# XuyangBai/PointDSC

Measured on NVIDIA H100. Metric: correspondence-sets/sec (PointDSC.forward, N=1000, B=256), higher is better.
Workload: dtype fp16 hi/lo split (3 products) with f32 accumulate

## Files before the change

pointdsc_b200/csrc/tc_attention.cuh:

```cuda
#pragma once
#include "tc_common.cuh"

namespace pdsc {

struct AttnArgs {
  int split;
  const uint8_t* qimg;
  const uint8_t* kvimg;
  const float* sc;
  float* msg;
  int items;
  float* part_o;
  float* part_ml;
  const SetDesc* sets;
  int nsets;
};

struct AttnItem {
  int N, QT, KT;
  int qt, t0, T;
  int sp;
  int qtile, kt0;
  int row0;
  long long sc0;
};

__device__ __forceinline__ AttnItem attn_item(const AttnArgs& a, int witem) {
  const SetDesc d = a.sets[find_set(a.nsets, witem, [&](int i) { return a.sets[i].item0; })];
  const int local = witem - d.item0;
  AttnItem w;
  w.N = d.N; w.QT = (d.N + 127) / 128; w.KT = (d.N + 63) / 64;
  w.qt = local / d.sp; w.t0 = (local % d.sp) * d.TS; w.T = d.TS; w.sp = d.sp;
  w.qtile = d.qt0 + w.qt; w.kt0 = d.kt0; w.row0 = d.row0; w.sc0 = d.sc0;
  return w;
}

constexpr int kAttnThreads = 384;
constexpr uint32_t kAttnConsumerRegs = 232, kAttnProducerRegs = 40;

__device__ __forceinline__ float ex2_approx(float x) {
  float y;
  asm("ex2.approx.ftz.f32 %0, %1;" : "=f"(y) : "f"(x));
  return y;
}
__device__ __forceinline__ float2 ldg_stream2(const float* p) {
  float2 v;
  asm volatile("ld.global.nc.L1::no_allocate.v2.f32 {%0, %1}, [%2];" : "=f"(v.x), "=f"(v.y) : "l"(p));
  return v;
}
__device__ __forceinline__ void attn_load_sc(float (&sc)[32], const float* tile, int r0, int fc) {
#pragma unroll
  for (int jj = 0; jj < 8; ++jj)
#pragma unroll
    for (int h = 0; h < 2; ++h) {
      const int key = 8 * jj + fc;
      const float2 v = ldg_stream2(tile + ((key >> 2) * 128 + r0 + 8 * h) * 4 + (key & 3));
      sc[4 * jj + 2 * h] = v.x;
      sc[4 * jj + 2 * h + 1] = v.y;
    }
}

}
```

pointdsc_b200/csrc/tc_attention_p.cuh:

```cuda
#pragma once
#include "tc_attention.cuh"

namespace pdsc {

constexpr int kAttnPQ = 0;
constexpr int kAttnPKV = 65536;
constexpr int kAttnStages = 2;
constexpr int kAttnPBars = kAttnPKV + kAttnStages * 65536;
constexpr int kAttnPSmem = kAttnPBars + 128;

template <int FMT>
__global__ void __launch_bounds__(kAttnThreads, 1) tc_attention_persistent_kernel(AttnArgs a) {
  extern __shared__ __align__(1024) uint8_t smem[];
  uint64_t* bars = reinterpret_cast<uint64_t*>(smem + kAttnPBars);
  const uint32_t s0 = smem_u32(smem);
  const uint32_t q_full = smem_u32(bars + 0), q_empty = smem_u32(bars + 1);
  const uint32_t kv_full = smem_u32(bars + 2), kv_empty = smem_u32(bars + 4);
  const int tid = threadIdx.x, warp = tid >> 5, lane = tid & 31;
  const int my_items = (a.items > (int)blockIdx.x) ? (a.items - (int)blockIdx.x + (int)gridDim.x - 1) / (int)gridDim.x : 0;

  if (tid == 0) {
    if (s0 & 1023u) __trap();
    mbar_init(q_full, 1);
    mbar_init(q_empty, 256);
    for (int i = 0; i < kAttnStages; ++i) {
      mbar_init(kv_full + 8 * i, 1);
      mbar_init(kv_empty + 8 * i, 256);
    }
    fence_barrier_init();
  }
  __syncthreads();

  if (warp >= 8) {
    setmaxnreg_dec<kAttnProducerRegs>();
    if (warp == 8 && lane == 0) {
      const uint32_t q_bytes = a.split ? 65536u : 32768u;
      const uint32_t tile_bytes = a.split ? 32768u : 16384u;
      int gt = 0;
      for (int it = 0; it < my_items; ++it) {
        const int witem = blockIdx.x + it * gridDim.x;
        const AttnItem w = attn_item(a, witem);
        if (it > 0) mbar_wait(q_empty, (uint32_t)((it - 1) & 1));
        mbar_expect_tx(q_full, q_bytes);
        for (uint32_t off = 0; off < q_bytes; off += 32768u)
          bulk_g2s(s0 + kAttnPQ + off, a.qimg + (size_t)w.qtile * 65536 + off, 32768u, q_full);
        for (int j = 0; j < w.T; ++j, ++gt) {
          const int st = gt % kAttnStages, use = gt / kAttnStages;
          if (use > 0) mbar_wait(kv_empty + 8 * st, (uint32_t)((use - 1) & 1));
          const int kt = min(w.t0 + j, w.KT - 1);
          const uint8_t* kv = a.kvimg + ((size_t)w.kt0 + kt) * 65536;
          const uint32_t dst = s0 + kAttnPKV + st * 65536;
          mbar_expect_tx(kv_full + 8 * st, 2 * tile_bytes);
          bulk_g2s(dst, kv, tile_bytes, kv_full + 8 * st);
          bulk_g2s(dst + 32768, kv + 32768, tile_bytes, kv_full + 8 * st);
        }
      }
    }
    __syncwarp();
    return;
  }

  setmaxnreg_inc<kAttnConsumerRegs>();
  const int wg = warp >> 2, wt = tid & 127;
  const int r0 = 64 * wg + frag_row(wt), fc = frag_col(wt);
  const uint32_t qa = s0 + kAttnPQ + (uint32_t)wg * 8192u;
  int gt = 0;
  for (int it = 0; it < my_items; ++it) {
    const int witem = blockIdx.x + it * gridDim.x;
    const AttnItem w = attn_item(a, witem);
    const int N = w.N, qt = w.qt, t0 = w.t0, T = w.T, KT = w.KT;
    const size_t tile_stride = (size_t)w.QT << 13;
    const float* sc_cta = a.sc + w.sc0 + ((size_t)qt << 13);
    float o[64];
#pragma unroll
    for (int i = 0; i < 64; ++i) o[i] = 0.f;
    float m[2] = {-INFINITY, -INFINITY}, l_sum[2] = {0.f, 0.f};
    float sc[32];
    attn_load_sc(sc, sc_cta + (size_t)min(t0, KT - 1) * tile_stride, r0, fc);
    mbar_wait(q_full, (uint32_t)(it & 1));
    for (int j = 0; j < T; ++j, ++gt) {
      const int st = gt % kAttnStages, use = gt / kAttnStages;
      const uint32_t kb = s0 + kAttnPKV + st * 65536, vb = kb + 32768;
      mbar_wait(kv_full + 8 * st, (uint32_t)(use & 1));
      float s[32];
      wgmma_fence();
      gemm_ss<FMT, 2, 64>(s, qa, qa + 32768, 16384, kb, kb + 16384, 8192, a.split);
      wgmma_commit();
      wgmma_wait<0>();
      fence_regs(s);
      if (j == T - 1) mbar_arrive(q_empty);
#pragma unroll
      for (int i = 0; i < 32; ++i) s[i] *= sc[i];
      if (j + 1 < T) attn_load_sc(sc, sc_cta + (size_t)min(t0 + j + 1, KT - 1) * tile_stride, r0, fc);
      if ((t0 + j) * 64 + 63 >= N) {
#pragma unroll
        for (int i = 0; i < 32; ++i)
          if ((t0 + j) * 64 + 8 * (i >> 2) + fc + (i & 1) >= N) s[i] = -INFINITY;
      }
      float scale[2];
#pragma unroll
      for (int h = 0; h < 2; ++h) {
        float tmax = -INFINITY;
#pragma unroll
        for (int jj = 0; jj < 8; ++jj) tmax = fmaxf(tmax, fmaxf(s[4 * jj + 2 * h], s[4 * jj + 2 * h + 1]));
        tmax = fmaxf(tmax, __shfl_xor_sync(0xffffffffu, tmax, 1));
        tmax = fmaxf(tmax, __shfl_xor_sync(0xffffffffu, tmax, 2));
        const float mn = fmaxf(m[h], tmax);
        scale[h] = (mn > m[h]) ? ex2_approx(m[h] - mn) : 1.0f;
        m[h] = mn;
        l_sum[h] *= scale[h];
      }
      float rsum[2] = {0.f, 0.f};
#pragma unroll
      for (int i = 0; i < 32; ++i) {
        const int h = (i >> 1) & 1;
        s[i] = ex2_approx(s[i] - m[h]);
        rsum[h] += s[i];
      }
      l_sum[0] += rsum[0];
      l_sum[1] += rsum[1];
#pragma unroll
      for (int i = 0; i < 64; ++i) o[i] *= scale[(i >> 1) & 1];
      uint32_t phi[4][4], plo[4][4];
      frag_split<FMT, 4>(s, phi, plo);
      wgmma_fence();
      gemm_rs<FMT, 4, 128, 1>(o, phi, plo, vb, vb + 16384, 8192, a.split, 1);
      wgmma_commit();
      wgmma_wait<0>();
      fence_regs(o);
      mbar_arrive(kv_empty + 8 * st);
    }
    const bool partial = w.sp > 1;
#pragma unroll
    for (int h = 0; h < 2; ++h) {
      float lt = l_sum[h];
      lt += __shfl_xor_sync(0xffffffffu, lt, 1);
      lt += __shfl_xor_sync(0xffffffffu, lt, 2);
      const int r = r0 + 8 * h;
      const float inv_l = partial ? 1.0f : 1.0f / lt;
      if (partial && (lane & 3) == 0) *reinterpret_cast<float2*>(a.part_ml + ((size_t)witem * 128 + r) * 2) = make_float2(m[h], lt);
      if (!partial && qt * 128 + r >= N) continue;
      float* dst = partial ? a.part_o + ((size_t)witem * 128 + r) * kC : a.msg + ((size_t)w.row0 + qt * 128 + r) * kC;
#pragma unroll
      for (int jj = 0; jj < 16; ++jj)
        *reinterpret_cast<float2*>(dst + 8 * jj + fc) = make_float2(o[4 * jj + 2 * h] * inv_l, o[4 * jj + 2 * h + 1] * inv_l);
    }
// ... 53 lines not shown
```

pointdsc_b200/csrc/encoder_tc.cu:

```cuda
#include <cuda_bf16.h>
#include <cuda_fp16.h>
#include <cuda_runtime.h>

#include <cmath>
#include <cstdlib>
#include <cstring>
#include <vector>

#include "common.cuh"
#include "encoder_tc.h"
#include "kernels.h"
#include "tc_attention.cuh"
#include "tc_attention_p.cuh"
#include "tc_chain.cuh"
#include "tc_common.cuh"
#include "tc_ptx.cuh"

namespace pdsc {

template <int FMT>
static void build_image(const float* W, int rows, int K, double scale, uint8_t* dst) {
  const int panels = K / 64;
  const size_t panel_bytes = (size_t)rows * 128;
  uint8_t* hi = dst;
// ... 86 lines not shown
  return split ? 1 : 0;
}

int tc_launches(int num_layers, int attn_split) {
  return 2 + (attn_split ? 5 : 4) * num_layers;
}

__global__ void tc_clear_pads_kernel(uint8_t* kvimg, const SetDesc* __restrict__ sets) {
  const int b = blockIdx.x;
  const SetDesc d = sets[b];
  const int first_pad = d.N & 63;
  if (first_pad == 0) return;
  uint8_t* base = kvimg + ((size_t)d.kt0 + (d.N + 63) / 64 - 1) * 65536;
  const int pads = 64 - first_pad;
  for (int t = threadIdx.x; t < pads * 128; t += blockDim.x) {
    const uint32_t n = (uint32_t)(first_pad + t / 128), c = (uint32_t)(t % 128);
    const uint32_t koff = (c >> 6) * 8192u + sw128_offset(n, c & 63u);
    *reinterpret_cast<uint16_t*>(base + koff) = 0;
    *reinterpret_cast<uint16_t*>(base + 16384 + koff) = 0;
    *reinterpret_cast<uint16_t*>(base + 32768 + koff) = 0;
    *reinterpret_cast<uint16_t*>(base + 49152 + koff) = 0;
  }
}

template <int FMT>
__global__ void tc_decode_kernel(const uint8_t* qimg, const uint8_t* kvimg, float* q, float* k, float* v, long long rows,
                                 const SetDesc* __restrict__ sets, int nsets, int split) {
  const long long idx = (long long)blockIdx.x * blockDim.x + threadIdx.x;
  const long long row = idx / kC;
  const uint32_t c = (uint32_t)(idx % kC);
  if (row >= rows) return;
  const SetDesc d = sets[find_set(nsets, row, [&](int i) { return sets[i].row0; })];
  const int n = (int)(row - d.row0);
  auto rd = [](const uint8_t* p) { return from_16<FMT>(*reinterpret_cast<const uint16_t*>(p)); };
  const uint8_t* qb = qimg + ((size_t)d.qt0 + (n >> 7)) * 65536;
  const uint32_t qo = (c >> 6) * 16384u + sw128_offset((uint32_t)(n & 127), c & 63u);
  q[idx] = rd(qb + qo) + (split ? rd(qb + 32768 + qo) : 0.f);
  const uint8_t* kb = kvimg + ((size_t)d.kt0 + (n >> 6)) * 65536;
  const uint32_t ko = (c >> 6) * 8192u + sw128_offset((uint32_t)(n & 63), c & 63u);
  k[idx] = rd(kb + ko) + (split ? rd(kb + 16384 + ko) : 0.f);
  v[idx] = rd(kb + 32768 + ko) + (split ? rd(kb + 49152 + ko) : 0.f);
}

__global__ void tc_unblock_f32_kernel(const float* __restrict__ blocked, float* __restrict__ plain, long long rows) {
  const long long i = (long long)blockIdx.x * blockDim.x + threadIdx.x;
  if (i >= rows * 32) return;
  const long long g = i >> 5;
  const uint32_t piece = (uint32_t)(i & 31);
  const float4 v = *reinterpret_cast<const float4*>(reinterpret_cast<const uint8_t*>(blocked) + blocked_f32_offset(g, piece));
  float* o = plain + 4 * i;
  o[0] = v.x; o[1] = v.y; o[2] = v.z; o[3] = v.w;
}

template <int FMT>
static cudaError_t tc_configure_fmt() {
  cudaError_t e;
  if ((e = ensure_dynamic_smem(reinterpret_cast<const void*>(tc_chain_kernel<kPCQ, FMT>), kChainSmem))) return e;
  if ((e = ensure_dynamic_smem(reinterpret_cast<const void*>(tc_chain_kernel<kKV, FMT>), kChainSmem))) return e;
  if ((e = ensure_dynamic_smem(reinterpret_cast<const void*>(tc_chain_kernel<kMSG, FMT>), kChainSmem))) return e;
  return ensure_dynamic_smem(reinterpret_cast<const void*>(tc_attention_persistent_kernel<FMT>), kAttnPSmem);
}

template <int FMT>
static int tc_encoder_forward_fmt(const TcWeights& w, const TcForwardArgs& a, cudaStream_t st) {
  const long long rows = a.rows;
  if (rows >= (1LL << 31)) return (int)cudaErrorInvalidValue;
  uint8_t* qimg = static_cast<uint8_t*>(a.scratch);
  qimg = reinterpret_cast<uint8_t*>((reinterpret_cast<uintptr_t>(qimg) + 1023) & ~uintptr_t(1023));
  uint8_t* kvimg = qimg + (size_t)a.qtiles * 65536;
  float* part_o = reinterpret_cast<float*>(kvimg + (size_t)a.ktiles * 65536);
  float* part_ml = part_o + partial_items(a.attn_invariant, a.attn_split, a.attn_items) * 128 * kC;
  const long long tiles = (rows + 127) / 128;
  const int num_sms = device_sm_count();
  if (num_sms <= 0) return (int)cudaErrorInvalidDevice;
  const int grid = (int)(tiles < num_sms ? tiles : num_sms);
  const uint8_t* arena = static_cast<const uint8_t*>(w.arena) + (size_t)FMT * w.num_layers * kLayerBytes;

  launch_layer0(a.corr_pos, a.l0w, a.l0b, a.feat, rows, a.in_dim, st);
  tc_clear_pads_kernel<<<a.nsets, 256, 0, st>>>(kvimg, a.sets);
  for (int l = 0; l < a.num_layers; ++l) {
    const uint8_t* base = arena + (size_t)l * kLayerBytes;
    ChainArgs c{};
    c.rows = rows; c.split = a.split;
    c.sets = a.sets; c.tile_set = a.tile_set; c.nsets = a.nsets;
    c.qimg = qimg; c.kvimg = kvimg; c.bias = reinterpret_cast<const float*>(base + kBias);
    c.in = a.feat; c.res = nullptr; c.out_f32 = a.feat1; c.wimg = base + kW1; c.wbytes = 131072;
    tc_chain_kernel<kPCQ, FMT><<<grid, kChainThreads, kChainSmem, st>>>(c);
    c.in = a.feat1; c.out_f32 = nullptr; c.wimg = base + kWk; c.wbytes = 131072;
    tc_chain_kernel<kKV, FMT><<<grid, kChainThreads, kChainSmem, st>>>(c);
    const AttnArgs at{a.split, qimg, kvimg, a.sc, a.msg, a.attn_items, part_o, part_ml, a.sets, a.nsets};
    if (a.attn_events) cudaEventRecord(a.attn_events[2 * l], st);
    tc_attention_persistent_kernel<FMT><<<at.items < num_sms ? at.items : num_sms, kAttnThreads, kAttnPSmem, st>>>(at);
    if (a.attn_split)
      tc_attention_merge_kernel<<<(unsigned)(a.qtiles * 4), 256, 0, st>>>(part_o, part_ml, a.msg, a.sets, a.nsets);
    if (a.attn_events) cudaEventRecord(a.attn_events[2 * l + 1], st);
    if (a.debug_out && a.debug_layer == l) {
      const size_t plane = (size_t)rows * kC;
      tc_unblock_f32_kernel<<<(unsigned)((plane / 4 + 255) / 256), 256, 0, st>>>(a.feat1, a.debug_out, rows);
      tc_decode_kernel<FMT><<<(unsigned)((plane + 255) / 256), 256, 0, st>>>(qimg, kvimg, a.debug_out + plane, a.debug_out + 2 * plane,
                                                                             a.debug_out + 3 * plane, rows, a.sets, a.nsets, a.split);
      cudaMemcpyAsync(a.debug_out + 4 * plane, a.msg, plane * sizeof(float), cudaMemcpyDeviceToDevice, st);
    }
    c.in = a.msg; c.res = a.feat1; c.out_f32 = a.feat; c.wimg = base + kWm0; c.wbytes = 81920;
    tc_chain_kernel<kMSG, FMT><<<grid, kChainThreads, kChainSmem, st>>>(c);
    if (a.layer_tap_out && a.layer_tap == l)
      cudaMemcpyAsync(a.layer_tap_out, a.feat, (size_t)rows * kC * sizeof(float), cudaMemcpyDeviceToDevice, st);
  }
  return (int)cudaGetLastError();
}

int tc_encoder_forward(const TcWeights& w, const TcForwardArgs& a, cudaStream_t st) {
  const cudaError_t e = a.fmt == kFmtBF16 ? tc_configure_fmt<kFmtBF16>() : tc_configure_fmt<kFmtF16>();
  if (e != cudaSuccess) return (int)e;
  return a.fmt == kFmtBF16 ? tc_encoder_forward_fmt<kFmtBF16>(w, a, st) : tc_encoder_forward_fmt<kFmtF16>(w, a, st);
}

}
```

pointdsc_b200/csrc/tc_chain.cuh:

```cuda
#pragma once
#include <climits>

#include "tc_common.cuh"

namespace pdsc {

constexpr int kChainThreads = 256;
constexpr int kChIn = 0;
constexpr int kChW = 65536;
constexpr int kChRes = kChW + 81920;
constexpr int kChBias = kChRes + 65536;
constexpr int kChBars = kChBias + 1024;
constexpr int kChainSmem = kChBars + 64;

struct SetWindow {
  int lo, row0, t0;
};
template <int MODE>
__device__ __forceinline__ SetWindow load_window(const ChainArgs& a, int lo) {
  const int lane = threadIdx.x & 31, w = min(lo + lane, a.nsets - 1);
  return {lo, lo + lane < a.nsets ? __ldg(&a.sets[w].row0) : INT_MAX, MODE == kPCQ ? __ldg(&a.sets[w].qt0) : __ldg(&a.sets[w].kt0)};
}

template <int MODE>
__device__ __forceinline__ void locate_row(const ChainArgs& a, const SetWindow& win, long long g, int& tile, int& r) {
  int k = 0;
#pragma unroll
  for (int s = 16; s > 0; s >>= 1)
    if (__shfl_sync(0xffffffffu, win.row0, k + s) <= g) k += s;
  int row0 = __shfl_sync(0xffffffffu, win.row0, k), t0 = __shfl_sync(0xffffffffu, win.t0, k);
  if (k == 31) {
    int b = win.lo + 31;
    while (b + 1 < a.nsets && __ldg(&a.sets[b + 1].row0) <= g) ++b;
    row0 = __ldg(&a.sets[b].row0);
    t0 = MODE == kPCQ ? __ldg(&a.sets[b].qt0) : __ldg(&a.sets[b].kt0);
  }
  const int nn = (int)(g - row0);
  tile = t0 + (MODE == kPCQ ? (nn >> 7) : (nn >> 6));
  r = MODE == kPCQ ? (nn & 127) : (nn & 63);
}

__host__ __device__ __forceinline__ size_t blocked_f32_offset(long long g, uint32_t piece) {
  return (size_t)(g >> 7) * 65536 + (size_t)(piece >> 3) * 16384 + (size_t)(g & 127) * 128 + (size_t)(((piece & 7u) ^ ((uint32_t)g & 7u)) << 4);
}

__device__ __forceinline__ void quad_transpose(uint32_t (&v)[4], int q) {
#pragma unroll
  for (int s = 1; s <= 2; s <<= 1)
#pragma unroll
    for (int k = 0; k < 4; ++k) {
      if (k & s) continue;
      const bool up = (q & s) != 0;
      const uint32_t r = __shfl_xor_sync(0xffffffffu, up ? v[k] : v[k + s], s);
      if (up) v[k] = r;
      else v[k + s] = r;
    }
}

__device__ __forceinline__ void store_row(uint8_t* img, uint32_t panel_bytes, uint32_t row, const uint32_t (&w)[16], int q, bool store) {
#pragma unroll
  for (int m = 0; m < 4; ++m) {
    uint32_t v[4] = {w[4 * m], w[4 * m + 1], w[4 * m + 2], w[4 * m + 3]};
    quad_transpose(v, q);
    const uint32_t j = 4u * m + q;
    if (store) *reinterpret_cast<uint4*>(img + (j >> 3) * panel_bytes + sw128_offset(row, 8u * (j & 7u))) = make_uint4(v[0], v[1], v[2], v[3]);
  }
}

template <int MODE, int FMT>
__global__ void __launch_bounds__(kChainThreads, 1) tc_chain_kernel(ChainArgs a) {
  extern __shared__ __align__(1024) uint8_t smem[];
  const uint8_t* stage = smem + kChIn;
  const uint8_t* resbuf = smem + kChRes;
  float* bias = reinterpret_cast<float*>(smem + kChBias);
  uint64_t* bars = reinterpret_cast<uint64_t*>(smem + kChBars);
  const uint32_t s0 = smem_u32(smem);
  const uint32_t bar_w = smem_u32(bars), bar_in = smem_u32(bars + 1), bar_res = smem_u32(bars + 2);
  const int tid = threadIdx.x;
  const int wg = tid >> 7, wt = tid & 127;
  const uint32_t w_base = s0 + kChW;
  constexpr int kBiasSrc = (MODE == kPCQ) ? kB1 : (MODE == kKV) ? kBk : kBm0;
  const long long rows = a.rows;
  const long long num_tiles = (rows + 127) / 128;

  auto issue_input = [&](long long t) {
    const long long left = rows - t * 128;
    const uint32_t bytes = (MODE == kKV || left >= 128) ? 65536u : (uint32_t)left * 512u;
    mbar_expect_tx(bar_in, bytes);
    bulk_g2s(s0 + kChIn, reinterpret_cast<const uint8_t*>(a.in) + (size_t)t * 65536, bytes, bar_in);
  };
  auto in_offset = [](int r, int c) -> uint32_t {
    return MODE == kKV ? (uint32_t)blocked_f32_offset(r, (uint32_t)c >> 2) + (c & 3) * 4 : (uint32_t)(r * kC + c) * 4u;
  };

  if (tid == 0) {
    if (s0 & 1023u) __trap();
    mbar_init(bar_w, 1);
    mbar_init(bar_in, 1);
    mbar_init(bar_res, 1);
    fence_barrier_init();
  }
  bias[tid] = a.bias[kBiasSrc + tid];
  __syncthreads();
  if (tid == 0) {
    mbar_expect_tx(bar_w, (uint32_t)a.wbytes);
    for (int off = 0; off < a.wbytes; off += 32768)
      bulk_g2s(w_base + off, a.wimg + off, (uint32_t)min(32768, a.wbytes - off), bar_w);
    if (blockIdx.x < num_tiles) issue_input(blockIdx.x);
  }
  mbar_wait(bar_w, 0);
  const int fr = 64 * wg + frag_row(wt), fc = frag_col(wt);
  const int quad = fc >> 1;

  SetWindow win_next{};
  int lo_after = 0;
  if (MODE != kMSG && blockIdx.x < num_tiles) {
    win_next = load_window<MODE>(a, __ldg(a.tile_set + blockIdx.x));
    if (blockIdx.x + gridDim.x < num_tiles) lo_after = __ldg(a.tile_set + blockIdx.x + gridDim.x);
  }
  uint32_t phase = 0;
  for (long long tile = blockIdx.x; tile < num_tiles; tile += gridDim.x, phase ^= 1u) {
    const long long row0 = tile * 128;
    const long long g[2] = {row0 + fr, row0 + fr + 8};
    int tl[2], tr[2];
    if (MODE != kMSG) {
      const SetWindow win = win_next;
      if (tile + gridDim.x < num_tiles) {
        win_next = load_window<MODE>(a, lo_after);
        if (tile + 2 * gridDim.x < num_tiles) lo_after = __ldg(a.tile_set + tile + 2 * gridDim.x);
      }
#pragma unroll
      for (int h = 0; h < 2; ++h) locate_row<MODE>(a, win, g[h] < rows ? g[h] : row0, tl[h], tr[h]);
    }
    uint32_t ahi[8][4], alo[8][4];
    mbar_wait(bar_in, phase);
    {
      float x[64];
#pragma unroll
      for (int j = 0; j < 16; ++j)
#pragma unroll
        for (int h = 0; h < 2; ++h) {
          const float2 v = *reinterpret_cast<const float2*>(stage + in_offset(fr + 8 * h, 8 * j + fc));
          x[4 * j + 2 * h] = v.x;
          x[4 * j + 2 * h + 1] = v.y;
        }
      frag_split<FMT, 8>(x, ahi, alo);
    }
    __syncthreads();
    if (tid == 0) {
      if (tile + gridDim.x < num_tiles) issue_input(tile + gridDim.x);
      if (MODE == kMSG) {
        mbar_expect_tx(bar_res, 65536u);
        bulk_g2s(s0 + kChRes, reinterpret_cast<const uint8_t*>(a.res) + (size_t)tile * 65536, 65536u, bar_res);
      }
    }

    if (MODE == kPCQ) {
      float x[64];
      wgmma_fence();
      gemm_rs<FMT, 8, 128, 0>(x, ahi, alo, w_base, w_base + 32768, 16384, a.split, 0);
      wgmma_commit();
      wgmma_wait<0>();
      fence_regs(x);
#pragma unroll
      for (int j = 0; j < 16; ++j)
#pragma unroll
        for (int h = 0; h < 2; ++h) {
          const int c = 8 * j + fc, e = 4 * j + 2 * h;
          x[e] = fmaxf(x[e] + bias[c], 0.f);
          x[e + 1] = fmaxf(x[e + 1] + bias[c + 1], 0.f);
          if (g[h] < rows)
            *reinterpret_cast<float2*>(reinterpret_cast<uint8_t*>(a.out_f32) + blocked_f32_offset(g[h], (uint32_t)c >> 2) + (c & 3) * 4) =
                make_float2(x[e], x[e + 1]);
        }
      frag_split<FMT, 8>(x, ahi, alo);
      float q[64];
      wgmma_fence();
      gemm_rs<FMT, 8, 128, 0>(q, ahi, alo, w_base + 65536, w_base + 65536 + 32768, 16384, a.split, 0);
      wgmma_commit();
      wgmma_wait<0>();
      fence_regs(q);
#pragma unroll
      for (int h = 0; h < 2; ++h) {
        uint8_t* img = a.qimg + (size_t)tl[h] * 65536;
        const uint32_t r = (uint32_t)tr[h];
        uint32_t hi[16], lo[16];
#pragma unroll
        for (int j = 0; j < 16; ++j) {
          const int c = 8 * j + fc, e = 4 * j + 2 * h;
          split_pair<FMT>(q[e] + bias[128 + c], q[e + 1] + bias[128 + c + 1], hi[j], lo[j]);
        }
        store_row(img, 16384u, r, hi, quad, g[h] < rows);
        if (a.split) store_row(img + 32768, 16384u, r, lo, quad, g[h] < rows);
      }
    } else if (MODE == kKV) {
#pragma unroll 1
      for (int step = 0; step < 2; ++step) {
        float x[64];
        const uint32_t wb = w_base + (uint32_t)step * 65536u;
        wgmma_fence();
        gemm_rs<FMT, 8, 128, 0>(x, ahi, alo, wb, wb + 32768, 16384, a.split, 0);
        wgmma_commit();
        wgmma_wait<0>();
        fence_regs(x);
        const float* bvec = bias + 128 * step;
#pragma unroll
        for (int h = 0; h < 2; ++h) {
          uint8_t* img = a.kvimg + (size_t)tl[h] * 65536 + 32768 * step;
          const uint32_t r = (uint32_t)tr[h];
          uint32_t hi[16], lo[16];
#pragma unroll
          for (int j = 0; j < 16; ++j) {
            const int c = 8 * j + fc, e = 4 * j + 2 * h;
            split_pair<FMT>(x[e] + bvec[c], x[e + 1] + bvec[c + 1], hi[j], lo[j]);
          }
          store_row(img, 8192u, r, hi, quad, g[h] < rows);
          if (a.split) store_row(img + 16384, 8192u, r, lo, quad, g[h] < rows);
        }
      }
    } else {
      float h0[32];
      wgmma_fence();
      gemm_rs<FMT, 8, 64, 0>(h0, ahi, alo, w_base, w_base + 16384, 8192, a.split, 0);
      wgmma_commit();
      wgmma_wait<0>();
      fence_regs(h0);
#pragma unroll
      for (int j = 0; j < 8; ++j)
#pragma unroll
        for (int e = 0; e < 4; ++e) h0[4 * j + e] = fmaxf(h0[4 * j + e] + bias[8 * j + fc + (e & 1)], 0.f);
      uint32_t bhi[4][4], blo[4][4];
      frag_split<FMT, 4>(h0, bhi, blo);
      float h1[32];
      wgmma_fence();
      gemm_rs<FMT, 4, 64, 0>(h1, bhi, blo, w_base + 32768, w_base + 32768 + 8192, 8192, a.split, 0);
      wgmma_commit();
      wgmma_wait<0>();
      fence_regs(h1);
#pragma unroll
      for (int j = 0; j < 8; ++j)
#pragma unroll
        for (int e = 0; e < 4; ++e) h1[4 * j + e] = fmaxf(h1[4 * j + e] + bias[64 + 8 * j + fc + (e & 1)], 0.f);
      frag_split<FMT, 4>(h1, bhi, blo);
      float o[64];
      wgmma_fence();
      gemm_rs<FMT, 4, 128, 0>(o, bhi, blo, w_base + 49152, w_base + 49152 + 16384, 16384, a.split, 0);
      wgmma_commit();
      wgmma_wait<0>();
      fence_regs(o);
      mbar_wait(bar_res, phase);
#pragma unroll
      for (int h = 0; h < 2; ++h) {
        if (g[h] >= rows) continue;
#pragma unroll
        for (int j = 0; j < 16; ++j) {
          const int c = 8 * j + fc, e = 4 * j + 2 * h;
          const float2 rv = *reinterpret_cast<const float2*>(resbuf + blocked_f32_offset(fr + 8 * h, (uint32_t)c >> 2) + (c & 3) * 4);
          *reinterpret_cast<float2*>(a.out_f32 + g[h] * kC + c) =
              make_float2(rv.x + (o[e] + bias[128 + c]), rv.y + (o[e + 1] + bias[128 + c + 1]));
        }
      }
    }
  }
}

}
```

pointdsc_b200/csrc/tc_common.cuh:

```cuda
#pragma once
#include "common.cuh"
#include "sets.cuh"
#include "tc_ptx.cuh"

namespace pdsc {
using namespace ptx;

constexpr size_t kW1 = 0, kWq = 65536, kWk = 131072, kWv = 196608, kWm0 = 262144, kWm1 = 294912, kWm2 = 311296,
                 kBias = 344064, kLayerBytes = 348160;
constexpr int kB1 = 0, kBq = 128, kBk = 256, kBv = 384, kBm0 = 512, kBm1 = 576, kBm2 = 640, kBiasFloats = 768;

constexpr float kQScale = 1.4426950408889634f / 11.313708498984761f;

enum ChainMode { kPCQ = 0, kKV = 1, kMSG = 2 };

struct ChainArgs {
  long long rows;
  int split;
  const SetDesc* sets;
  const int* tile_set;
  int nsets;
  const float* in;
  const float* res;
  float* out_f32;
  uint8_t* qimg;
  uint8_t* kvimg;
  const uint8_t* wimg;
  const float* bias;
  int wbytes;
};


template <int FMT, int KP, int NOUT>
__device__ __forceinline__ void gemm_ss(float (&d)[NOUT / 2], uint32_t a_hi, uint32_t a_lo, uint32_t a_panel_bytes, uint32_t b_hi,
                                        uint32_t b_lo, uint32_t b_panel_bytes, int split) {
  uint32_t acc = 0;
#pragma unroll
  for (int t = 0; t < 3; ++t) {
    if (t > 0 && !split) break;
    const uint32_t a = (t == 2) ? a_lo : a_hi;
    const uint32_t b = (t == 1) ? b_lo : b_hi;
#pragma unroll
    for (int p = 0; p < KP; ++p) {
#pragma unroll
      for (int ks = 0; ks < 4; ++ks) {
        const uint64_t ad = smem_desc_sw128(a + p * a_panel_bytes + ks * 32);
        const uint64_t bd = smem_desc_sw128(b + p * b_panel_bytes + ks * 32);
        if constexpr (NOUT == 64) wgmma_ss_n64<FMT, 0>(d, ad, bd, acc);
        else wgmma_ss_n128<FMT, 0>(d, ad, bd, acc);
        acc = 1;
      }
    }
  }
}

template <int FMT, int KS, int NOUT, int TB>
__device__ __forceinline__ void gemm_rs(float (&d)[NOUT / 2], const uint32_t (&a_hi)[KS][4], const uint32_t (&a_lo)[KS][4], uint32_t b_hi,
                                        uint32_t b_lo, uint32_t b_panel_bytes, int split, uint32_t accumulate) {
  uint32_t acc = accumulate;
#pragma unroll
  for (int t = 0; t < 3; ++t) {
    if (t > 0 && !split) break;
    const uint32_t b = (t == 1) ? b_lo : b_hi;
#pragma unroll
    for (int ks = 0; ks < KS; ++ks) {
      const uint64_t bd = TB ? smem_desc_sw128(b + ks * 2048, b_panel_bytes)
                             : smem_desc_sw128(b + (ks >> 2) * b_panel_bytes + (ks & 3) * 32);
      if constexpr (NOUT == 64) wgmma_rs_n64<FMT, TB>(d, t == 2 ? a_lo[ks] : a_hi[ks], bd, acc);
      else wgmma_rs_n128<FMT, TB>(d, t == 2 ? a_lo[ks] : a_hi[ks], bd, acc);
      acc = 1;
    }
  }
}

template <int FMT, int KS>
__device__ __forceinline__ void frag_split(const float (&x)[8 * KS], uint32_t (&hi)[KS][4], uint32_t (&lo)[KS][4]) {
#pragma unroll
  for (int ks = 0; ks < KS; ++ks)
#pragma unroll
    for (int i = 0; i < 4; ++i) split_pair<FMT>(x[8 * ks + 2 * i], x[8 * ks + 2 * i + 1], hi[ks][i], lo[ks][i]);
}

// ... 5 lines not shown
```

pointdsc_b200/csrc/tc_ptx.cuh:

```cuda
#pragma once
#include <cuda_bf16.h>
#include <cuda_fp16.h>
#include <cuda_runtime.h>
#include <stdint.h>

#include <cstdio>

namespace pdsc {
namespace ptx {

__device__ __forceinline__ uint32_t smem_u32(const void* p) { return (uint32_t)__cvta_generic_to_shared(p); }

__device__ __forceinline__ void mbar_init(uint32_t bar, uint32_t count) {
  asm volatile("mbarrier.init.shared::cta.b64 [%0], %1;" ::"r"(bar), "r"(count) : "memory");
}
__device__ __forceinline__ void fence_barrier_init() {
  asm volatile("fence.mbarrier_init.release.cluster;" ::: "memory");
}
__device__ __forceinline__ void mbar_arrive(uint32_t bar) {
  asm volatile("mbarrier.arrive.shared::cta.b64 _, [%0];" ::"r"(bar) : "memory");
}
__device__ __forceinline__ void mbar_expect_tx(uint32_t bar, uint32_t bytes) {
  asm volatile("mbarrier.arrive.expect_tx.shared::cta.b64 _, [%0], %1;" ::"r"(bar), "r"(bytes) : "memory");
}
// ... 6 lines not shown
  asm volatile(
      "{\n\t.reg .pred p;\n\t"
      "mbarrier.try_wait.parity.shared::cta.b64 p, [%1], %2, %3;\n\t"
      "selp.u32 %0, 1, 0, p;\n\t}"
      : "=r"(ok)
      : "r"(bar), "r"(parity), "r"(kMbarSuspendHintNs)
      : "memory");
  return ok != 0;
}
__device__ __forceinline__ bool mbar_test(uint32_t bar, uint32_t parity) {
  uint32_t ok;
  asm volatile(
      "{\n\t.reg .pred p;\n\t"
      "mbarrier.test_wait.parity.shared::cta.b64 p, [%1], %2;\n\t"
      "selp.u32 %0, 1, 0, p;\n\t}"
      : "=r"(ok)
      : "r"(bar), "r"(parity)
      : "memory");
  return ok != 0;
}
__device__ __forceinline__ void mbar_wait(uint32_t bar, uint32_t parity) {
  if (mbar_try_wait(bar, parity)) return;
  const long long t0 = clock64();
  for (uint32_t tries = 1;; ++tries) {
    if (mbar_try_wait(bar, parity)) return;
    if ((tries & 63u) == 0u && clock64() - t0 > 8000000000LL) __trap();
  }
}

__device__ __forceinline__ void bulk_g2s(uint32_t dst_smem, const void* src_gmem, uint32_t bytes, uint32_t bar) {
  asm volatile("cp.async.bulk.shared::cluster.global.mbarrier::complete_tx::bytes [%0], [%1], %2, [%3];" ::"r"(dst_smem),
               "l"(src_gmem), "r"(bytes), "r"(bar)
               : "memory");
}

__device__ __forceinline__ void bulk_s2g(void* dst_gmem, uint32_t src_smem, uint32_t bytes) {
  asm volatile("cp.async.bulk.global.shared::cta.bulk_group [%0], [%1], %2;" ::"l"(__cvta_generic_to_global(dst_gmem)), "r"(src_smem),
               "r"(bytes)
               : "memory");
}
__device__ __forceinline__ void bulk_commit() { asm volatile("cp.async.bulk.commit_group;" ::: "memory"); }
template <int N>
__device__ __forceinline__ void bulk_wait_read() { asm volatile("cp.async.bulk.wait_group.read %0;" ::"n"(N) : "memory"); }
template <int N>
__device__ __forceinline__ void bulk_wait_all() { asm volatile("cp.async.bulk.wait_group %0;" ::"n"(N) : "memory"); }

template <uint32_t R>
__device__ __forceinline__ void setmaxnreg_dec() { asm volatile("setmaxnreg.dec.sync.aligned.u32 %0;" ::"n"(R)); }
template <uint32_t R>
__device__ __forceinline__ void setmaxnreg_inc() { asm volatile("setmaxnreg.inc.sync.aligned.u32 %0;" ::"n"(R)); }

__device__ __forceinline__ void fence_proxy_async_smem() { asm volatile("fence.proxy.async.shared::cta;" ::: "memory"); }

constexpr int kFmtF16 = 0, kFmtBF16 = 1;

template <int FMT>
__device__ __forceinline__ void split_pair(float a, float b, uint32_t& hi, uint32_t& lo) {
  if (FMT == kFmtBF16) {
    const __nv_bfloat162 h = __floats2bfloat162_rn(a, b);
    const float2 f = __bfloat1622float2(h);
    const __nv_bfloat162 l = __floats2bfloat162_rn(a - f.x, b - f.y);
    hi = *reinterpret_cast<const uint32_t*>(&h);
    lo = *reinterpret_cast<const uint32_t*>(&l);
  } else {
    const __half2 h = __floats2half2_rn(a, b);
    const float2 f = __half22float2(h);
    const __half2 l = __floats2half2_rn(a - f.x, b - f.y);
    hi = *reinterpret_cast<const uint32_t*>(&h);
    lo = *reinterpret_cast<const uint32_t*>(&l);
  }
}
template <int FMT>
__host__ __device__ __forceinline__ uint16_t to_16(float x) {
  if (FMT == kFmtBF16) {
    const __nv_bfloat16 h = __float2bfloat16_rn(x);
    return *reinterpret_cast<const uint16_t*>(&h);
  } else {
    const __half h = __float2half_rn(x);
    return *reinterpret_cast<const uint16_t*>(&h);
  }
}
template <int FMT>
__host__ __device__ __forceinline__ float from_16(uint16_t b) {
  if (FMT == kFmtBF16) {
    return __bfloat162float(*reinterpret_cast<const __nv_bfloat16*>(&b));
  } else {
    return __half2float(*reinterpret_cast<const __half*>(&b));
  }
}

__device__ __forceinline__ uint64_t smem_desc_sw128(uint32_t smem_addr, uint32_t lbo_bytes = 16u) {
  return (uint64_t)((smem_addr >> 4) & 0x3FFFu) | ((uint64_t)((lbo_bytes >> 4) & 0x3FFFu) << 16) | (64ull << 32) | (1ull << 62);
}
__device__ __forceinline__ void wgmma_fence() { asm volatile("wgmma.fence.sync.aligned;" ::: "memory"); }
__device__ __forceinline__ void wgmma_commit() { asm volatile("wgmma.commit_group.sync.aligned;" ::: "memory"); }
template <int N>
__device__ __forceinline__ void wgmma_wait() { asm volatile("wgmma.wait_group.sync.aligned %0;" ::"n"(N) : "memory"); }
template <int R>
__device__ __forceinline__ void fence_regs(float (&d)[R]) {
#pragma unroll
  for (int i = 0; i < R; ++i) asm volatile("" : "+f"(d[i])::"memory");
}

template <int FMT, int TB>
__device__ __forceinline__ void wgmma_ss_n64(float (&d)[32], uint64_t adesc, uint64_t bdesc, uint32_t accumulate) {
  if constexpr (FMT == kFmtBF16) {
// ... 73 lines not shown
```

Baseline: 15950.

## Exploit symmetric SC matrix: read transposed tiles and add L2 eviction hints

Attention now reads spatial-consistency tiles only from the lower block-triangle. Upper-triangle tiles are reconstructed by loading the transposed tile with scalar loads, relying on the matrix being symmetric. Loads carry L2 cache-policy hints: evict_last for tiles that will be re-read in transposed form, evict_first otherwise. The aim is to cut DRAM traffic for the large SC matrix, at the cost of less coalesced scalar loads on the transposed path. It is also correct only if the SC matrix is truly symmetric.

After: 16240, median of 6. 1.02x the previous value.

```diff
diff --git a/pointdsc_b200/csrc/tc_attention.cuh b/pointdsc_b200/csrc/tc_attention.cuh
--- a/pointdsc_b200/csrc/tc_attention.cuh
+++ b/pointdsc_b200/csrc/tc_attention.cuh
@@ -43,21 +43,50 @@
   asm("ex2.approx.ftz.f32 %0, %1;" : "=f"(y) : "f"(x));
   return y;
 }
-__device__ __forceinline__ float2 ldg_stream2(const float* p) {
+struct ScPolicy {
+  uint64_t keep, stream;
+};
+__device__ __forceinline__ ScPolicy sc_policy() {
+  ScPolicy p;
+  asm volatile("createpolicy.fractional.L2::evict_last.b64 %0, 1.0;" : "=l"(p.keep));
+  asm volatile("createpolicy.fractional.L2::evict_first.b64 %0, 1.0;" : "=l"(p.stream));
+  return p;
+}
+__device__ __forceinline__ float2 ldg_sc2(const float* p, uint64_t pol) {
   float2 v;
-  asm volatile("ld.global.nc.L1::no_allocate.v2.f32 {%0, %1}, [%2];" : "=f"(v.x), "=f"(v.y) : "l"(p));
+  asm volatile("ld.global.nc.L1::no_allocate.L2::cache_hint.v2.f32 {%0, %1}, [%2], %3;" : "=f"(v.x), "=f"(v.y) : "l"(p), "l"(pol));
   return v;
 }
-__device__ __forceinline__ void attn_load_sc(float (&sc)[32], const float* tile, int r0, int fc) {
+__device__ __forceinline__ float ldg_sc1(const float* p, uint64_t pol) {
+  float v;
+  asm volatile("ld.global.nc.L2::cache_hint.f32 %0, [%1], %2;" : "=f"(v) : "l"(p), "l"(pol));
+  return v;
+}
+
+__device__ __forceinline__ void attn_load_sc(float (&sc)[32], const float* sc_set, int QT, int qt, int kt, int r0, int fc,
+                                             const ScPolicy& pol) {
+  if ((kt >> 1) <= qt) {
+    const float* tile = sc_set + (((size_t)kt * QT + qt) << 13) + (fc >> 2) * 512 + r0 * 4 + (fc & 3);
+    const uint64_t p = (kt >> 1) < qt ? pol.keep : pol.stream;
 #pragma unroll
-  for (int jj = 0; jj < 8; ++jj)
+    for (int jj = 0; jj < 8; ++jj)
 #pragma unroll
-    for (int h = 0; h < 2; ++h) {
-      const int key = 8 * jj + fc;
-      const float2 v = ldg_stream2(tile + ((key >> 2) * 128 + r0 + 8 * h) * 4 + (key & 3));
-      sc[4 * jj + 2 * h] = v.x;
-      sc[4 * jj + 2 * h + 1] = v.y;
-    }
+      for (int h = 0; h < 2; ++h) {
+        const float2 v = ldg_sc2(tile + jj * 1024 + h * 32, p);
+        sc[4 * jj + 2 * h] = v.x;
+        sc[4 * jj + 2 * h + 1] = v.y;
+      }
+  } else {
+    const int k = r0 & 63;
+    const float* tile = sc_set + (((size_t)(2 * qt + (r0 >> 6)) * QT + (kt >> 1)) << 13) + (k >> 2) * 512 + (k & 3) +
+                        (64 * (kt & 1) + fc) * 4;
+#pragma unroll
+    for (int jj = 0; jj < 8; ++jj)
+#pragma unroll
+      for (int h = 0; h < 2; ++h)
+#pragma unroll
+        for (int e = 0; e < 2; ++e) sc[4 * jj + 2 * h + e] = ldg_sc1(tile + h * 1024 + (8 * jj + e) * 4, pol.stream);
+  }
 }
 
 }
diff --git a/pointdsc_b200/csrc/tc_attention_p.cuh b/pointdsc_b200/csrc/tc_attention_p.cuh
--- a/pointdsc_b200/csrc/tc_attention_p.cuh
+++ b/pointdsc_b200/csrc/tc_attention_p.cuh
@@ -64,19 +64,19 @@
   const int wg = warp >> 2, wt = tid & 127;
   const int r0 = 64 * wg + frag_row(wt), fc = frag_col(wt);
   const uint32_t qa = s0 + kAttnPQ + (uint32_t)wg * 8192u;
+  const ScPolicy pol = sc_policy();
   int gt = 0;
   for (int it = 0; it < my_items; ++it) {
     const int witem = blockIdx.x + it * gridDim.x;
     const AttnItem w = attn_item(a, witem);
     const int N = w.N, qt = w.qt, t0 = w.t0, T = w.T, KT = w.KT;
-    const size_t tile_stride = (size_t)w.QT << 13;
-    const float* sc_cta = a.sc + w.sc0 + ((size_t)qt << 13);
+    const float* sc_set = a.sc + w.sc0;
     float o[64];
 #pragma unroll
     for (int i = 0; i < 64; ++i) o[i] = 0.f;
     float m[2] = {-INFINITY, -INFINITY}, l_sum[2] = {0.f, 0.f};
     float sc[32];
-    attn_load_sc(sc, sc_cta + (size_t)min(t0, KT - 1) * tile_stride, r0, fc);
+    attn_load_sc(sc, sc_set, w.QT, qt, min(t0, KT - 1), r0, fc, pol);
     mbar_wait(q_full, (uint32_t)(it & 1));
     for (int j = 0; j < T; ++j, ++gt) {
       const int st = gt % kAttnStages, use = gt / kAttnStages;
@@ -91,7 +91,7 @@
       if (j == T - 1) mbar_arrive(q_empty);
 #pragma unroll
       for (int i = 0; i < 32; ++i) s[i] *= sc[i];
-      if (j + 1 < T) attn_load_sc(sc, sc_cta + (size_t)min(t0 + j + 1, KT - 1) * tile_stride, r0, fc);
+      if (j + 1 < T) attn_load_sc(sc, sc_set, w.QT, qt, min(t0 + j + 1, KT - 1), r0, fc, pol);
       if ((t0 + j) * 64 + 63 >= N) {
 #pragma unroll
         for (int i = 0; i < 32; ++i)
```

## Fuse next layer's first FC into message chain and enable programmatic dependent launch

Applied to the files above, without the earlier changes.

For every layer except the last, the message-FC chain kernel now also applies the next layer's first FC (W1 plus ReLU) and writes the blocked feature directly. The next layer then runs a Q-only chain instead of recomputing the first FC, which removes one kernel launch and one round trip of the feature tensor through global memory per layer. Chain kernels are launched with programmatic stream serialization and griddepcontrol, so weight prefetch and barrier setup overlap the tail of the previous kernel. In exchange the fused kernel loads more weights into shared memory, and the residual tile is staged in the input buffer, which makes the input prefetch wait until after the epilogue.

Measured after the change: 16030 before, 16620 after, median of 6. +3.7%, better.

```diff
diff --git a/pointdsc_b200/csrc/encoder_tc.cu b/pointdsc_b200/csrc/encoder_tc.cu
--- a/pointdsc_b200/csrc/encoder_tc.cu
+++ b/pointdsc_b200/csrc/encoder_tc.cu
@@ -162,12 +162,29 @@
   o[0] = v.x; o[1] = v.y; o[2] = v.z; o[3] = v.w;
 }
 
+template <int MODE, int FMT>
+static void launch_chain(int grid, const ChainArgs& c, cudaStream_t st) {
+  cudaLaunchConfig_t cfg{};
+  cfg.gridDim = dim3((unsigned)grid);
+  cfg.blockDim = dim3(kChainThreads);
+  cfg.dynamicSmemBytes = kChainSmem;
+  cfg.stream = st;
+  cudaLaunchAttribute attr[1];
+  attr[0].id = cudaLaunchAttributeProgrammaticStreamSerialization;
+  attr[0].val.programmaticStreamSerializationAllowed = 1;
+  cfg.attrs = attr;
+  cfg.numAttrs = 1;
+  cudaLaunchKernelEx(&cfg, tc_chain_kernel<MODE, FMT>, c);
+}
+
 template <int FMT>
 static cudaError_t tc_configure_fmt() {
   cudaError_t e;
   if ((e = ensure_dynamic_smem(reinterpret_cast<const void*>(tc_chain_kernel<kPCQ, FMT>), kChainSmem))) return e;
   if ((e = ensure_dynamic_smem(reinterpret_cast<const void*>(tc_chain_kernel<kKV, FMT>), kChainSmem))) return e;
   if ((e = ensure_dynamic_smem(reinterpret_cast<const void*>(tc_chain_kernel<kMSG, FMT>), kChainSmem))) return e;
+  if ((e = ensure_dynamic_smem(reinterpret_cast<const void*>(tc_chain_kernel<kMSGPC, FMT>), kChainSmem))) return e;
+  if ((e = ensure_dynamic_smem(reinterpret_cast<const void*>(tc_chain_kernel<kQ, FMT>), kChainSmem))) return e;
   return ensure_dynamic_smem(reinterpret_cast<const void*>(tc_attention_persistent_kernel<FMT>), kAttnPSmem);
 }
 
@@ -190,14 +207,20 @@
   tc_clear_pads_kernel<<<a.nsets, 256, 0, st>>>(kvimg, a.sets);
   for (int l = 0; l < a.num_layers; ++l) {
     const uint8_t* base = arena + (size_t)l * kLayerBytes;
+    const bool last = l + 1 == a.num_layers;
     ChainArgs c{};
     c.rows = rows; c.split = a.split;
     c.sets = a.sets; c.tile_set = a.tile_set; c.nsets = a.nsets;
     c.qimg = qimg; c.kvimg = kvimg; c.bias = reinterpret_cast<const float*>(base + kBias);
-    c.in = a.feat; c.res = nullptr; c.out_f32 = a.feat1; c.wimg = base + kW1; c.wbytes = 131072;
-    tc_chain_kernel<kPCQ, FMT><<<grid, kChainThreads, kChainSmem, st>>>(c);
+    if (l == 0) {
+      c.in = a.feat; c.out_f32 = a.feat1; c.wimg = base + kW1; c.wbytes = 131072;
+      launch_chain<kPCQ, FMT>(grid, c, st);
+    } else {
+      c.in = a.feat1; c.out_f32 = nullptr; c.wimg = base + kWq; c.wbytes = 65536;
+      launch_chain<kQ, FMT>(grid, c, st);
+    }
     c.in = a.feat1; c.out_f32 = nullptr; c.wimg = base + kWk; c.wbytes = 131072;
-    tc_chain_kernel<kKV, FMT><<<grid, kChainThreads, kChainSmem, st>>>(c);
+    launch_chain<kKV, FMT>(grid, c, st);
     const AttnArgs at{a.split, qimg, kvimg, a.sc, a.msg, a.attn_items, part_o, part_ml, a.sets, a.nsets};
     if (a.attn_events) cudaEventRecord(a.attn_events[2 * l], st);
     tc_attention_persistent_kernel<FMT><<<at.items < num_sms ? at.items : num_sms, kAttnThreads, kAttnPSmem, st>>>(at);
@@ -211,9 +234,18 @@
                                                                              a.debug_out + 3 * plane, rows, a.sets, a.nsets, a.split);
       cudaMemcpyAsync(a.debug_out + 4 * plane, a.msg, plane * sizeof(float), cudaMemcpyDeviceToDevice, st);
     }
-    c.in = a.msg; c.res = a.feat1; c.out_f32 = a.feat; c.wimg = base + kWm0; c.wbytes = 81920;
-    tc_chain_kernel<kMSG, FMT><<<grid, kChainThreads, kChainSmem, st>>>(c);
-    if (a.layer_tap_out && a.layer_tap == l)
+    const bool tap = a.layer_tap_out && a.layer_tap == l;
+    c.in = a.msg; c.res = a.feat1; c.wimg = base + kWm0; c.wbytes = 81920;
+    if (last) {
+      c.out_f32 = a.feat;
+      launch_chain<kMSG, FMT>(grid, c, st);
+    } else {
+      const uint8_t* next = base + kLayerBytes;
+      c.out_f32 = a.feat1; c.feat_out = tap ? a.feat : nullptr;
+      c.wimg1 = next + kW1; c.bias1 = reinterpret_cast<const float*>(next + kBias);
+      launch_chain<kMSGPC, FMT>(grid, c, st);
+    }
+    if (tap)
       cudaMemcpyAsync(a.layer_tap_out, a.feat, (size_t)rows * kC * sizeof(float), cudaMemcpyDeviceToDevice, st);
   }
   return (int)cudaGetLastError();
diff --git a/pointdsc_b200/csrc/tc_chain.cuh b/pointdsc_b200/csrc/tc_chain.cuh
--- a/pointdsc_b200/csrc/tc_chain.cuh
+++ b/pointdsc_b200/csrc/tc_chain.cuh
@@ -10,8 +10,11 @@
 constexpr int kChW = 65536;
 constexpr int kChRes = kChW + 81920;
 constexpr int kChBias = kChRes + 65536;
-constexpr int kChBars = kChBias + 1024;
+constexpr int kChBars = kChBias + 1536;
 constexpr int kChainSmem = kChBars + 64;
+
+template <int MODE>
+constexpr bool kWritesQ = MODE == kPCQ || MODE == kQ;
 
 struct SetWindow {
   int lo, row0, t0;
@@ -19,7 +22,7 @@
 template <int MODE>
 __device__ __forceinline__ SetWindow load_window(const ChainArgs& a, int lo) {
   const int lane = threadIdx.x & 31, w = min(lo + lane, a.nsets - 1);
-  return {lo, lo + lane < a.nsets ? __ldg(&a.sets[w].row0) : INT_MAX, MODE == kPCQ ? __ldg(&a.sets[w].qt0) : __ldg(&a.sets[w].kt0)};
+  return {lo, lo + lane < a.nsets ? __ldg(&a.sets[w].row0) : INT_MAX, kWritesQ<MODE> ? __ldg(&a.sets[w].qt0) : __ldg(&a.sets[w].kt0)};
 }
 
 template <int MODE>
@@ -33,11 +36,11 @@
     int b = win.lo + 31;
     while (b + 1 < a.nsets && __ldg(&a.sets[b + 1].row0) <= g) ++b;
     row0 = __ldg(&a.sets[b].row0);
-    t0 = MODE == kPCQ ? __ldg(&a.sets[b].qt0) : __ldg(&a.sets[b].kt0);
+    t0 = kWritesQ<MODE> ? __ldg(&a.sets[b].qt0) : __ldg(&a.sets[b].kt0);
   }
   const int nn = (int)(g - row0);
-  tile = t0 + (MODE == kPCQ ? (nn >> 7) : (nn >> 6));
-  r = MODE == kPCQ ? (nn & 127) : (nn & 63);
+  tile = t0 + (kWritesQ<MODE> ? (nn >> 7) : (nn >> 6));
+  r = kWritesQ<MODE> ? (nn & 127) : (nn & 63);
 }
 
 __host__ __device__ __forceinline__ size_t blocked_f32_offset(long long g, uint32_t piece) {
@@ -79,20 +82,23 @@
   const int tid = threadIdx.x;
   const int wg = tid >> 7, wt = tid & 127;
   const uint32_t w_base = s0 + kChW;
-  constexpr int kBiasSrc = (MODE == kPCQ) ? kB1 : (MODE == kKV) ? kBk : kBm0;
+  constexpr bool kFcMsg = MODE == kMSG || MODE == kMSGPC;
+  constexpr bool kBlockedIn = MODE == kKV || MODE == kQ;
+  constexpr int kBiasSrc = (MODE == kPCQ) ? kB1 : (MODE == kQ) ? kBq : (MODE == kKV) ? kBk : kBm0;
   const long long rows = a.rows;
   const long long num_tiles = (rows + 127) / 128;
 
   auto issue_input = [&](long long t) {
     const long long left = rows - t * 128;
-    const uint32_t bytes = (MODE == kKV || left >= 128) ? 65536u : (uint32_t)left * 512u;
+    const uint32_t bytes = (kBlockedIn || left >= 128) ? 65536u : (uint32_t)left * 512u;
     mbar_expect_tx(bar_in, bytes);
     bulk_g2s(s0 + kChIn, reinterpret_cast<const uint8_t*>(a.in) + (size_t)t * 65536, bytes, bar_in);
   };
   auto in_offset = [](int r, int c) -> uint32_t {
-    return MODE == kKV ? (uint32_t)blocked_f32_offset(r, (uint32_t)c >> 2) + (c & 3) * 4 : (uint32_t)(r * kC + c) * 4u;
+    return kBlockedIn ? (uint32_t)blocked_f32_offset(r, (uint32_t)c >> 2) + (c & 3) * 4 : (uint32_t)(r * kC + c) * 4u;
   };
 
+  griddep_launch_dependents();
   if (tid == 0) {
     if (s0 & 1023u) __trap();
     mbar_init(bar_w, 1);
@@ -101,20 +107,24 @@
     fence_barrier_init();
   }
   bias[tid] = a.bias[kBiasSrc + tid];
+  if (MODE == kMSGPC && tid < 128) bias[256 + tid] = a.bias1[kB1 + tid];
   __syncthreads();
   if (tid == 0) {
-    mbar_expect_tx(bar_w, (uint32_t)a.wbytes);
+    mbar_expect_tx(bar_w, (uint32_t)a.wbytes + (MODE == kMSGPC ? 65536u : 0u));
     for (int off = 0; off < a.wbytes; off += 32768)
       bulk_g2s(w_base + off, a.wimg + off, (uint32_t)min(32768, a.wbytes - off), bar_w);
-    if (blockIdx.x < num_tiles) issue_input(blockIdx.x);
-  }
+    if (MODE == kMSGPC)
+      for (int off = 0; off < 65536; off += 32768) bulk_g2s(s0 + kChRes + off, a.wimg1 + off, 32768u, bar_w);
+  }
+  griddep_wait();
+  if (tid == 0 && blockIdx.x < num_tiles) issue_input(blockIdx.x);
   mbar_wait(bar_w, 0);
   const int fr = 64 * wg + frag_row(wt), fc = frag_col(wt);
   const int quad = fc >> 1;
 
   SetWindow win_next{};
   int lo_after = 0;
-  if (MODE != kMSG && blockIdx.x < num_tiles) {
+  if (!kFcMsg && blockIdx.x < num_tiles) {
     win_next = load_window<MODE>(a, __ldg(a.tile_set + blockIdx.x));
     if (blockIdx.x + gridDim.x < num_tiles) lo_after = __ldg(a.tile_set + blockIdx.x + gridDim.x);
   }
@@ -123,7 +133,7 @@
     const long long row0 = tile * 128;
     const long long g[2] = {row0 + fr, row0 + fr + 8};
     int tl[2], tr[2];
-    if (MODE != kMSG) {
+    if (!kFcMsg) {
       const SetWindow win = win_next;
       if (tile + gridDim.x < num_tiles) {
         win_next = load_window<MODE>(a, lo_after);
@@ -148,35 +158,39 @@
     }
     __syncthreads();
     if (tid == 0) {
-      if (tile + gridDim.x < num_tiles) issue_input(tile + gridDim.x);
-      if (MODE == kMSG) {
+      if (MODE != kMSGPC && tile + gridDim.x < num_tiles) issue_input(tile + gridDim.x);
+      if (kFcMsg) {
         mbar_expect_tx(bar_res, 65536u);
-        bulk_g2s(s0 + kChRes, reinterpret_cast<const uint8_t*>(a.res) + (size_t)tile * 65536, 65536u, bar_res);
-      }
-    }
-
-    if (MODE == kPCQ) {
-      float x[64];
-      wgmma_fence();
-      gemm_rs<FMT, 8, 128, 0>(x, ahi, alo, w_base, w_base + 32768, 16384, a.split, 0);
-      wgmma_commit();
-      wgmma_wait<0>();
-      fence_regs(x);
-#pragma unroll
-      for (int j = 0; j < 16; ++j)
-#pragma unroll
-        for (int h = 0; h < 2; ++h) {
-          const int c = 8 * j + fc, e = 4 * j + 2 * h;
-          x[e] = fmaxf(x[e] + bias[c], 0.f);
-          x[e + 1] = fmaxf(x[e + 1] + bias[c + 1], 0.f);
-          if (g[h] < rows)
-            *reinterpret_cast<float2*>(reinterpret_cast<uint8_t*>(a.out_f32) + blocked_f32_offset(g[h], (uint32_t)c >> 2) + (c & 3) * 4) =
-                make_float2(x[e], x[e + 1]);
-        }
-      frag_split<FMT, 8>(x, ahi, alo);
+        bulk_g2s(s0 + (MODE == kMSG ? kChRes : kChIn), reinterpret_cast<const uint8_t*>(a.res) + (size_t)tile * 65536, 65536u, bar_res);
+      }
+    }
+
+    if (kWritesQ<MODE>) {
+      if (MODE == kPCQ) {
+        float x[64];
+        wgmma_fence();
+        gemm_rs<FMT, 8, 128, 0>(x, ahi, alo, w_base, w_base + 32768, 16384, a.split, 0);
+        wgmma_commit();
+        wgmma_wait<0>();
+        fence_regs(x);
+#pragma unroll
+        for (int j = 0; j < 16; ++j)
+#pragma unroll
+          for (int h = 0; h < 2; ++h) {
+            const int c = 8 * j + fc, e = 4 * j + 2 * h;
+            x[e] = fmaxf(x[e] + bias[c], 0.f);
+            x[e + 1] = fmaxf(x[e + 1] + bias[c + 1], 0.f);
+            if (g[h] < rows)
+              *reinterpret_cast<float2*>(reinterpret_cast<uint8_t*>(a.out_f32) + blocked_f32_offset(g[h], (uint32_t)c >> 2) + (c & 3) * 4) =
+                  make_float2(x[e], x[e + 1]);
+          }
+        frag_split<FMT, 8>(x, ahi, alo);
+      }
+      const uint32_t wq = w_base + (MODE == kPCQ ? 65536u : 0u);
+      const float* bq = bias + (MODE == kPCQ ? 128 : 0);
       float q[64];
       wgmma_fence();
-      gemm_rs<FMT, 8, 128, 0>(q, ahi, alo, w_base + 65536, w_base + 65536 + 32768, 16384, a.split, 0);
+      gemm_rs<FMT, 8, 128, 0>(q, ahi, alo, wq, wq + 32768, 16384, a.split, 0);
       wgmma_commit();
       wgmma_wait<0>();
       fence_regs(q);
@@ -188,7 +202,7 @@
 #pragma unroll
         for (int j = 0; j < 16; ++j) {
           const int c = 8 * j + fc, e = 4 * j + 2 * h;
-          split_pair<FMT>(q[e] + bias[128 + c], q[e + 1] + bias[128 + c + 1], hi[j], lo[j]);
+          split_pair<FMT>(q[e] + bq[c], q[e + 1] + bq[c + 1], hi[j], lo[j]);
         }
         store_row(img, 16384u, r, hi, quad, g[h] < rows);
         if (a.split) store_row(img + 32768, 16384u, r, lo, quad, g[h] < rows);
@@ -248,20 +262,52 @@
       wgmma_commit();
       wgmma_wait<0>();
       fence_regs(o);
-      mbar_wait(bar_res, phase);
-#pragma unroll
-      for (int h = 0; h < 2; ++h) {
-        if (g[h] >= rows) continue;
-#pragma unroll
-        for (int j = 0; j < 16; ++j) {
-          const int c = 8 * j + fc, e = 4 * j + 2 * h;
-          const float2 rv = *reinterpret_cast<const float2*>(resbuf + blocked_f32_offset(fr + 8 * h, (uint32_t)c >> 2) + (c & 3) * 4);
-          *reinterpret_cast<float2*>(a.out_f32 + g[h] * kC + c) =
-              make_float2(rv.x + (o[e] + bias[128 + c]), rv.y + (o[e + 1] + bias[128 + c + 1]));
+      if (MODE == kMSG) {
+        mbar_wait(bar_res, phase);
+#pragma unroll
+        for (int h = 0; h < 2; ++h) {
+          if (g[h] >= rows) continue;
+#pragma unroll
+          for (int j = 0; j < 16; ++j) {
+            const int c = 8 * j + fc, e = 4 * j + 2 * h;
+            const float2 rv = *reinterpret_cast<const float2*>(resbuf + blocked_f32_offset(fr + 8 * h, (uint32_t)c >> 2) + (c & 3) * 4);
+            *reinterpret_cast<float2*>(a.out_f32 + g[h] * kC + c) =
+                make_float2(rv.x + (o[e] + bias[128 + c]), rv.y + (o[e + 1] + bias[128 + c + 1]));
+          }
         }
-      }
-    }
-  }
-}
-
-}
+      } else {
+        mbar_wait(bar_res, phase);
+#pragma unroll
+        for (int j = 0; j < 16; ++j)
+#pragma unroll
+          for (int h = 0; h < 2; ++h) {
+            const int c = 8 * j + fc, e = 4 * j + 2 * h;
+            const float2 rv = *reinterpret_cast<const float2*>(stage + blocked_f32_offset(fr + 8 * h, (uint32_t)c >> 2) + (c & 3) * 4);
+            o[e] = rv.x + (o[e] + bias[128 + c]);
+            o[e + 1] = rv.y + (o[e + 1] + bias[128 + c + 1]);
+            if (a.feat_out && g[h] < rows) *reinterpret_cast<float2*>(a.feat_out + g[h] * kC + c) = make_float2(o[e], o[e + 1]);
+          }
+        __syncthreads();
+        if (tid == 0 && tile + gridDim.x < num_tiles) issue_input(tile + gridDim.x);
+        frag_split<FMT, 8>(o, ahi, alo);
+        float x[64];
+        wgmma_fence();
+        gemm_rs<FMT, 8, 128, 0>(x, ahi, alo, s0 + kChRes, s0 + kChRes + 32768, 16384, a.split, 0);
+        wgmma_commit();
+        wgmma_wait<0>();
+        fence_regs(x);
+#pragma unroll
+        for (int j = 0; j < 16; ++j)
+#pragma unroll
+          for (int h = 0; h < 2; ++h) {
+            const int c = 8 * j + fc, e = 4 * j + 2 * h;
+            if (g[h] < rows)
+              *reinterpret_cast<float2*>(reinterpret_cast<uint8_t*>(a.out_f32) + blocked_f32_offset(g[h], (uint32_t)c >> 2) + (c & 3) * 4) =
+                  make_float2(fmaxf(x[e] + bias[256 + c], 0.f), fmaxf(x[e + 1] + bias[256 + c + 1], 0.f));
+          }
+      }
+    }
+  }
+}
+
+}
diff --git a/pointdsc_b200/csrc/tc_common.cuh b/pointdsc_b200/csrc/tc_common.cuh
--- a/pointdsc_b200/csrc/tc_common.cuh
+++ b/pointdsc_b200/csrc/tc_common.cuh
@@ -12,7 +12,7 @@
 
 constexpr float kQScale = 1.4426950408889634f / 11.313708498984761f;
 
-enum ChainMode { kPCQ = 0, kKV = 1, kMSG = 2 };
+enum ChainMode { kPCQ = 0, kKV = 1, kMSG = 2, kMSGPC = 3, kQ = 4 };
 
 struct ChainArgs {
   long long rows;
@@ -23,11 +23,14 @@
   const float* in;
   const float* res;
   float* out_f32;
+  float* feat_out;
   uint8_t* qimg;
   uint8_t* kvimg;
   const uint8_t* wimg;
   const float* bias;
   int wbytes;
+  const uint8_t* wimg1;
+  const float* bias1;
 };
 
 
diff --git a/pointdsc_b200/csrc/tc_ptx.cuh b/pointdsc_b200/csrc/tc_ptx.cuh
--- a/pointdsc_b200/csrc/tc_ptx.cuh
+++ b/pointdsc_b200/csrc/tc_ptx.cuh
@@ -82,6 +82,9 @@
 
 __device__ __forceinline__ void fence_proxy_async_smem() { asm volatile("fence.proxy.async.shared::cta;" ::: "memory"); }
 
+__device__ __forceinline__ void griddep_launch_dependents() { asm volatile("griddepcontrol.launch_dependents;" ::: "memory"); }
+__device__ __forceinline__ void griddep_wait() { asm volatile("griddepcontrol.wait;" ::: "memory"); }
+
 constexpr int kFmtF16 = 0, kFmtBF16 = 1;
 
 template <int FMT>
```
